# apachepinot/pinot

Hardware: AMD Instinct MI355X
Metric: rows scanned/sec, 1B-row segment filter+groupby (3 predicates, SUM/MAX GROUP BY g1) (higher is better)
Workload: dtype int64; 1 GPU; 1 segment(s) x 1000000000 rows, one per GPU; SELECT g1, SUM(m), MAX(m) FROM gpuBench WHERE c_inv1 IN (0,1,2,3) AND c_inv2 IN (0,1) AND r_int BETWEEN 250000 AND 749999 GROUP BY g1 ORDER BY g1 LIMIT 1000; query=cfg3, parallelism=segment-per-gpu x1, merge=none (1 segment), entries_scanned_in_filter=249990290

## Files before the change

pinot_amd/csrc/pg_kernels_spec.hip:

```cpp
#define PG_WAVES_PER_BLOCK 12
#define PG_KERNEL template <int PG_NOT_INSTANTIATED> static
#include "pg_kernels.hip"

#define SPEC_LOADERS 4
#ifndef SPEC_TILES
#define SPEC_TILES 2
#endif
#ifndef SPEC_SETS
#define SPEC_SETS 2
#endif
#define SPEC_CONSUMERS 8
#define SPEC_OFF_LIN 0u
#define SPEC_OFF_RNG 256u
#define SPEC_OFF_VAL (256u + 2048u)
#define SPEC_OFF_G0 (256u + 2048u + 8192u)
extern "C" const int pg_spec_waves_per_block = PG_WAVES_PER_BLOCK;
extern "C" int pg_spec_stage_bytes(int bits0, int bits1) { return SPEC_TILES * (((int)SPEC_OFF_G0 + bits0 * 256 + 16 + (bits1 > 0 ? bits1 * 256 + 16 : 0) + 15) & ~15); }

DEVFN void spec_barrier() {
  __builtin_amdgcn_fence(__ATOMIC_RELEASE, "workgroup", "local");
  __builtin_amdgcn_s_barrier();
  __builtin_amdgcn_fence(__ATOMIC_ACQUIRE, "workgroup", "local");
}

template <typename T> DEVFN const GAS T* spec_sgpr_ptr(const void* ptr) {
  const uint64_t v = (uint64_t)ptr;
  const uint32_t lo = (uint32_t)__builtin_amdgcn_readfirstlane((int)(uint32_t)v), hi = (uint32_t)__builtin_amdgcn_readfirstlane((int)(uint32_t)(v >> 32));
  return (const GAS T*)(((uint64_t)hi << 32) | (uint64_t)lo);
}

template <int W> struct SpecCol;
template <> struct SpecCol<0> {};
template <> struct SpecCol<32> { u32x4 r[2]; };
template <> struct SpecCol<24> { u32x4 lo; u32x2 hi; };
template <> struct SpecCol<16> { u32x4 lo; };
template <> struct SpecCol<8> { u32x2 hi; };
constexpr uint32_t spec_img_tile_bytes(int W) { return (uint32_t)(PG_WAVE_DOCS / 8) * (uint32_t)W; }
template <int W> DEVFN void spec_load(SpecCol<W>& c, const uint8_t* base, int wt, int w, int lane) {
  if constexpr (W == 32) {
#pragma unroll
    for (int s = 0; s < 2; s++) {
      const uint8_t* row = base + (size_t)wt * (PG_WAVE_DOCS * 4) + (size_t)(4 * s + w) * 1024u;
      c.r[s] = ldnt((const GAS u32x4*)(spec_sgpr_ptr<uint8_t>(row) + (uint32_t)lane * 16u));
    }
  } else if constexpr (W != 0) {
    const uint8_t* tile = base + (size_t)wt * spec_img_tile_bytes(W);
    if constexpr (W >= 16) c.lo = ldnt((const GAS u32x4*)(spec_sgpr_ptr<uint8_t>(tile + (size_t)w * 1024u) + (uint32_t)lane * 16u));
    if constexpr (W != 16) c.hi = ldnt((const GAS u32x2*)(spec_sgpr_ptr<uint8_t>(tile + (W == 24 ? 4096u : 0u) + (size_t)w * 512u) + (uint32_t)lane * 8u));
  }
}
template <int W> DEVFN void spec_unpack(const SpecCol<W>& c, uint32_t (&a)[4], uint32_t (&b)[4]) {
  if constexpr (W == 32) {
    a[0] = bswap32(c.r[0].x); a[1] = bswap32(c.r[0].y); a[2] = bswap32(c.r[0].z); a[3] = bswap32(c.r[0].w);
    b[0] = bswap32(c.r[1].x); b[1] = bswap32(c.r[1].y); b[2] = bswap32(c.r[1].z); b[3] = bswap32(c.r[1].w);
  } else if constexpr (W == 24) {
    a[0] = __builtin_amdgcn_perm(c.hi.x, c.lo.x, 0x0c040100u); a[1] = __builtin_amdgcn_perm(c.hi.x, c.lo.x, 0x0c050302u);
    a[2] = __builtin_amdgcn_perm(c.hi.x, c.lo.y, 0x0c060100u); a[3] = __builtin_amdgcn_perm(c.hi.x, c.lo.y, 0x0c070302u);
    b[0] = __builtin_amdgcn_perm(c.hi.y, c.lo.z, 0x0c040100u); b[1] = __builtin_amdgcn_perm(c.hi.y, c.lo.z, 0x0c050302u);
    b[2] = __builtin_amdgcn_perm(c.hi.y, c.lo.w, 0x0c060100u); b[3] = __builtin_amdgcn_perm(c.hi.y, c.lo.w, 0x0c070302u);
  } else if constexpr (W == 16) {
    a[0] = c.lo.x & 0xFFFFu; a[1] = c.lo.x >> 16; a[2] = c.lo.y & 0xFFFFu; a[3] = c.lo.y >> 16;
    b[0] = c.lo.z & 0xFFFFu; b[1] = c.lo.z >> 16; b[2] = c.lo.w & 0xFFFFu; b[3] = c.lo.w >> 16;
  } else if constexpr (W == 8) {
#pragma unroll
    for (int e = 0; e < 4; e++) { a[e] = (c.hi.x >> (8 * e)) & 0xFFu; b[e] = (c.hi.y >> (8 * e)) & 0xFFu; }
  }
}
template <int SW, int VW> struct SpecTile {
  SpecCol<SW> scan;
  SpecCol<VW> val;
  u32x4 grp;
};
template <int SW, int VW> struct SpecStage { SpecTile<SW, VW> tile[SPEC_TILES]; uint32_t post[8]; uint32_t tail; };
template <int NG> struct SpecQuad {
  uint32_t lin, rng;
  u32x4 val;
  uint32_t win[NG][2];
};

template <int W> struct SpecWidth { static constexpr int value = W; };
template <int NG, bool HAS_INDEX, bool HAS_SCAN, bool HAS_TAIL = false, bool NARROW = false>
__device__ __forceinline__ void spec_body(const PgQueryPlan& p) {
  extern __shared__ __attribute__((aligned(16))) uint64_t smem[];
  __shared__ uint32_t s_stat[PG_MAX_STATS];
  const int t = threadIdx.x;
  const int lane = t & 63;
  const int wave = uniform(t >> 6);
  int64_t* lds_table = reinterpret_cast<int64_t*>(smem);
  if (t < PG_MAX_STATS) s_stat[t] = 0;
  const uint32_t real_slots = (uint32_t)p.n_groups * (uint32_t)p.replicas;
  const uint32_t table_slots = real_slots + 64u;
  for (int o = 0; o < p.n_ops; o++) {
    const int64_t ident = pg_acc_identity(p.ops[o].fn, p.ops[o].is_float);
    for (uint32_t i = t; i < table_slots; i += PG_BLOCK) lds_table[(size_t)o * table_slots + i] = ident;
  }
  const uint32_t bits0 = (uint32_t)p.gcols[0].bits, bits1 = NG > 1 ? (uint32_t)p.gcols[NG - 1].bits : 0u;
  const uint32_t off_g1 = SPEC_OFF_G0 + bits0 * 256u + 16u;
  const uint32_t tile_bytes = (off_g1 + (NG > 1 ? bits1 * 256u + 16u : 0u) + 15u) & ~15u;
  const uint32_t stage_bytes = tile_bytes * SPEC_TILES;
  uint8_t* stage0 = reinterpret_cast<uint8_t*>(smem) + (((size_t)p.n_ops * table_slots * 8u + 15u) & ~(size_t)15u);
  const CAS PgScanLeaf& L = cptr(p.scans)[HAS_SCAN ? p.fast_scan : 0];
  const int grid = (int)gridDim.x;
  const int n_mine = (int)blockIdx.x < p.n_wtiles ? (p.n_wtiles - (int)blockIdx.x + grid - 1) / grid : 0;
  const int n_stages = (n_mine + SPEC_TILES - 1) / SPEC_TILES;
  __syncthreads();

  if (wave < SPEC_LOADERS) {
    const int w = wave;
    const uint8_t* const xdata = p.srcs[p.pipe_src].data;
    const uint8_t* const simg = NARROW ? p.spec_simg : nullptr;
    const uint8_t* const vimg = NARROW ? p.spec_vimg : nullptr;
    const uint32_t img_slo = NARROW ? p.spec_slo : 0u, img_sspan = NARROW ? p.spec_sspan : 0u, img_vmin = NARROW ? (uint32_t)p.spec_vmin : 0u;
    const bool img_sempty = NARROW && p.spec_sempty != 0;
    const int ggi = (w >> 1) < NG ? (w >> 1) : 0;
    const uint8_t* const gdata = p.gcols[ggi].data;
    const uint32_t gbits = (uint32_t)p.gcols[ggi].bits;
    const uint32_t goff = (uint32_t)(w & 1) * 1024u + (uint32_t)lane * 16u;
    const uint32_t geff = (w >> 1) < NG && goff < gbits * 256u ? goff : 0u;
    const uint8_t* dense_ptr[8];
    int dense_group[8];
#pragma unroll
    for (int j = 0; j < 8; j++) { dense_ptr[j] = HAS_INDEX ? p.dense_ptr[j] : nullptr; dense_group[j] = HAS_INDEX ? p.dense_group[j] : 0; }
    const int dense_groups = p.dense_groups, dense_excl = p.dense_excl;
    const uint8_t* const pipe_tail = HAS_TAIL ? p.pipe_tail : nullptr;
    const int num_docs = p.num_docs;
    const bool scan_pushed = p.fast_scan_pushed != 0;
   auto loaders = [&](auto scan_w, auto val_w) __attribute__((always_inline)) {
    constexpr int SW = HAS_SCAN ? decltype(scan_w)::value : 0, VW = decltype(val_w)::value;
    const RangeI32 r32 = !HAS_SCAN ? RangeI32{0, 0u, false} : (SW == 32 ? make_range_i32(L.lo, L.hi) : RangeI32{(int32_t)img_slo, img_sspan, img_sempty});
    const uint8_t* sdata = !HAS_SCAN ? nullptr : (SW == 32 ? L.data : simg);
    const uint8_t* vdata = VW == 32 ? xdata : vimg;
    const uint32_t vmin = VW == 32 ? 0u : img_vmin;
    uint32_t ld_cand = 0;
    auto issue = [&](int sidx, SpecStage<SW, VW>& st) __attribute__((always_inline)) {
#pragma unroll
      for (int tt = 0; tt < SPEC_TILES; tt++) {
        const int i = sidx * SPEC_TILES + tt;
        const int wt = (int)blockIdx.x + (i < n_mine ? i : n_mine - 1) * grid;
        SpecTile<SW, VW>& tl = st.tile[tt];
        __builtin_amdgcn_sched_barrier(0);
        spec_load<SW>(tl.scan, sdata, wt, w, lane);
        spec_load<VW>(tl.val, vdata, wt, w, lane);
        __builtin_amdgcn_sched_barrier(0);
        {
          const uint8_t* base = gdata + (size_t)wt * (size_t)(PG_WAVE_DOCS / 8) * (size_t)gbits;
          tl.grp = ldnt((const GAS u32x4*)(spec_sgpr_ptr<uint8_t>(base) + geff));
        }
        __builtin_amdgcn_sched_barrier(0);
      }
      if (HAS_INDEX) {
        const int i = sidx * SPEC_TILES + (w % SPEC_TILES);
        const int wt = (int)blockIdx.x + (i < n_mine ? i : n_mine - 1) * grid;
#pragma unroll
        for (int j = 0; j < 8; j++) st.post[j] = *(const GAS uint32_t*)(spec_sgpr_ptr<uint8_t>(dense_ptr[j] + (size_t)wt * 256u) + (uint32_t)lane * 4u);
        __builtin_amdgcn_sched_barrier(0);
      }
      if (HAS_TAIL) {
        const int i = sidx * SPEC_TILES + (w % SPEC_TILES);
        const int wt = (int)blockIdx.x + (i < n_mine ? i : n_mine - 1) * grid;
        st.tail = *(const GAS uint32_t*)(spec_sgpr_ptr<uint8_t>(pipe_tail + (size_t)wt * 256u) + (uint32_t)lane * 4u);
        __builtin_amdgcn_sched_barrier(0);
      }
    };
    auto publish = [&](uint8_t* stage, const SpecStage<SW, VW>& st) __attribute__((always_inline)) {
#ifdef PG_SPEC_NO_PUBLISH
      {
        uint32_t acc = 0;
#pragma unroll
        for (int tt = 0; tt < SPEC_TILES; tt++) {
          uint32_t a[4] = {0u, 0u, 0u, 0u}, b[4] = {0u, 0u, 0u, 0u};
          spec_unpack<SW>(st.tile[tt].scan, a, b); acc += a[0] ^ b[3];
          spec_unpack<VW>(st.tile[tt].val, a, b); acc += a[0] ^ b[3];
          acc += st.tile[tt].grp.x;
        }
        if (acc == 0x12345678u) *reinterpret_cast<uint32_t*>(stage) = acc;
        return;
      }
#endif
#pragma unroll
      for (int tt = 0; tt < SPEC_TILES; tt++) {
        uint8_t* buf = stage + (uint32_t)tt * tile_bytes;
        const SpecTile<SW, VW>& tl = st.tile[tt];
        if (HAS_SCAN) {
          uint32_t q[2][4];
          spec_unpack<SW>(tl.scan, q[0], q[1]);
#pragma unroll
          for (int s = 0; s < 2; s++) {
            uint32_t m = (uint32_t)in_range_i32(r32, (int32_t)q[s][0]) | ((uint32_t)in_range_i32(r32, (int32_t)q[s][1]) << 1) |
                         ((uint32_t)in_range_i32(r32, (int32_t)q[s][2]) << 2) | ((uint32_t)in_range_i32(r32, (int32_t)q[s][3]) << 3);
            m = r32.empty ? 0u : m;
            *reinterpret_cast<uint32_t*>(buf + SPEC_OFF_RNG + (uint32_t)(4 * s + w) * 256u + (uint32_t)lane * 4u) = m;
          }
        }
        {
          uint32_t q[2][4];
          spec_unpack<VW>(tl.val, q[0], q[1]);
#pragma unroll
          for (int s = 0; s < 2; s++) {
            u32x4 v;
            v.x = q[s][0] + vmin; v.y = q[s][1] + vmin; v.z = q[s][2] + vmin; v.w = q[s][3] + vmin;
            *reinterpret_cast<u32x4*>(buf + SPEC_OFF_VAL + (uint32_t)(4 * s + w) * 1024u + (uint32_t)lane * 16u) = v;
          }
        }
        *reinterpret_cast<u32x4*>(buf + (ggi == 0 ? SPEC_OFF_G0 : off_g1) + geff) = tl.grp;
      }
    };
    auto publish_lin = [&](uint8_t* stage, const SpecStage<SW, VW>& st, int sidx) __attribute__((always_inline)) {
      if (w >= SPEC_TILES) return;
      const int i = sidx * SPEC_TILES + w;
      const int wt = (int)blockIdx.x + i * grid;
      const int64_t rem = i < n_mine ? (int64_t)num_docs - (int64_t)wt * PG_WAVE_DOCS : 0;
      const int32_t n_valid = rem >= PG_WAVE_DOCS ? PG_WAVE_DOCS : (rem > 0 ? (int32_t)rem : 0);
      uint32_t lin = valid_lin_mask(n_valid, lane);
      if (HAS_INDEX) {
        uint32_t grp[4] = {0u, 0u, 0u, 0u};
#pragma unroll
        for (int j = 0; j < 8; j++) {
          const int gj = dense_group[j];
#pragma unroll
          for (int k = 0; k < 4; k++) grp[k] |= gj == k ? st.post[j] : 0u;
        }
#pragma unroll
        for (int k = 0; k < 4; k++)
          if (k < dense_groups) lin &= ((dense_excl >> k) & 1) ? ~grp[k] : grp[k];
      }
      *reinterpret_cast<uint32_t*>(stage + (uint32_t)w * tile_bytes + SPEC_OFF_LIN + (uint32_t)lane * 4u) = HAS_TAIL ? lin & st.tail : lin;
      ld_cand += (uint32_t)__popc(lin);
    };
    constexpr int SETS = HAS_SCAN ? SPEC_SETS : 2 * SPEC_SETS;
    SpecStage<SW, VW> st[SETS];
    auto buf_of = [&](int sg) __attribute__((always_inline)) { return stage0 + (uint32_t)(sg & 1) * stage_bytes; };
    if (n_stages > 0) {
#pragma unroll
      for (int k = 0; k < SETS; k++) issue(k, st[k]);
    }
    int s = 0;
    for (; s + SETS - 1 < n_stages; s += SETS) {
#pragma unroll
      for (int k = 0; k < SETS; k++) {
        publish(buf_of(s + k), st[k]);
        publish_lin(buf_of(s + k), st[k], s + k);
        issue(s + k + SETS, st[k]);
        spec_barrier();
      }
    }
#pragma unroll
    for (int k = 0; k < SETS - 1; k++)
      if (s + k < n_stages) {
        publish(buf_of(s + k), st[k]);
        publish_lin(buf_of(s + k), st[k], s + k);
        spec_barrier();
      }
    const uint32_t csum = wave_sum_u32(ld_cand);
    if (HAS_SCAN && !scan_pushed && lane == 0 && csum) atomicAdd(&s_stat[L.stat_slot], csum);
   };
    if constexpr (!NARROW) {
      loaders(SpecWidth<32>{}, SpecWidth<32>{});
    } else {
      const int sb = uniform(p.spec_sbits), vb = uniform(p.spec_vbits);
      auto with_scan = [&](auto scan_w) __attribute__((always_inline)) {
        switch (vb) {
          case 8: loaders(scan_w, SpecWidth<8>{}); break;
          case 16: loaders(scan_w, SpecWidth<16>{}); break;
          case 24: loaders(scan_w, SpecWidth<24>{}); break;
          default: loaders(scan_w, SpecWidth<32>{}); break;
        }
      };
      switch (sb) {
        case 8: with_scan(SpecWidth<8>{}); break;
        case 16: with_scan(SpecWidth<16>{}); break;
        case 24: with_scan(SpecWidth<24>{}); break;
        default: with_scan(SpecWidth<32>{}); break;
      }
    }
  } else {
    const int c = wave - SPEC_LOADERS;
    const uint32_t R = (uint32_t)p.replicas;
    const uint32_t rep = (uint32_t)t & (R - 1u);
    const uint32_t stride = table_slots;
    const uint32_t trash_slot = real_slots + (uint32_t)lane;
    const uint32_t q = (uint32_t)c * 64u + (uint32_t)lane;
    const uint32_t nib = ((uint32_t)lane & 7u) * 4u;
    uint32_t my_matched = 0;
    const int n_ops = uniform(p.n_ops);
    uint64_t ops_code = 0;
    for (int o = 0; o < n_ops; o++) {
      const PgAccOp op = p.ops[uniform(o)];
      ops_code |= (uint64_t)(op.src < 0 ? 0u : (op.fn == PG_ACC_SUM ? 1u : (op.fn == PG_ACC_MIN ? 2u : 3u))) << (2 * o);
    }
    ops_code = ((uint64_t)(uint32_t)uniform((int)(uint32_t)(ops_code >> 32)) << 32) | (uint64_t)(uint32_t)uniform((int)(uint32_t)ops_code);
    const int has_out_words = uniform(p.out_words != nullptr ? 1 : 0);
    auto fetch = [&](const uint8_t* buf, SpecQuad<NG>& d) __attribute__((always_inline)) {
      d.lin = *reinterpret_cast<const uint32_t*>(buf + SPEC_OFF_LIN + (q >> 3) * 4u);
      d.rng = HAS_SCAN ? *reinterpret_cast<const uint32_t*>(buf + SPEC_OFF_RNG + q * 4u) : 0xFu;
      d.val = *reinterpret_cast<const u32x4*>(buf + SPEC_OFF_VAL + q * 16u);
#pragma unroll
      for (int gi = 0; gi < NG; gi++) {
        const uint32_t di = __umul24(4u * q, (uint32_t)p.gcols[gi].bits) >> 5;
        const uint32_t* win = reinterpret_cast<const uint32_t*>(buf + (gi == 0 ? SPEC_OFF_G0 : off_g1)) + di;
        d.win[gi][0] = win[0]; d.win[gi][1] = win[1];
      }
    };
    auto aggregate = [&](const SpecQuad<NG> (&d)[SPEC_TILES], int sidx) __attribute__((always_inline)) {
      constexpr int ND = 4 * SPEC_TILES;
      uint32_t slot[ND];
      int32_t v[ND];
#pragma unroll
      for (int tt = 0; tt < SPEC_TILES; tt++) {
        const int i = sidx * SPEC_TILES + tt;
        const uint32_t cand = (d[tt].lin >> nib) & 0xFu;
        const uint32_t m = d[tt].rng & cand;
        my_matched += (uint32_t)__popc(m);
        if (has_out_words && i < n_mine) {
          const int wt = (int)blockIdx.x + i * grid;
          const uint32_t word = or_reduce8(m << nib);
          if ((lane & 7) == 0) reinterpret_cast<uint32_t*>(p.out_words)[(int64_t)wt * 64 + (int64_t)(q >> 3)] = word;
        }
#ifndef PG_SPEC_NO_TABLE
#pragma unroll
        for (int e = 0; e < 4; e++) slot[4 * tt + e] = rep;
#pragma unroll
        for (int gi = 0; gi < NG; gi++) {
          const PgGroupCol& gc = p.gcols[gi];
          const uint32_t bits = (uint32_t)gc.bits, mask = (1u << gc.bits) - 1u;
          const uint32_t mult = (uint32_t)gc.mult * R;
          uint32_t dv[4];
          decode_packed_quad<true>(d[tt].win[gi], q, bits, mask, dv);
#pragma unroll
          for (int e = 0; e < 4; e++) slot[4 * tt + e] += __umul24(dv[e], mult);
        }
#pragma unroll
        for (int e = 0; e < 4; e++) slot[4 * tt + e] = ((m >> e) & 1u) ? slot[4 * tt + e] : trash_slot;
        v[4 * tt + 0] = (int32_t)d[tt].val.x; v[4 * tt + 1] = (int32_t)d[tt].val.y; v[4 * tt + 2] = (int32_t)d[tt].val.z; v[4 * tt + 3] = (int32_t)d[tt].val.w;
#endif
      }
#ifdef PG_SPEC_NO_TABLE
      return;
#endif
      for (int o = 0; o < n_ops; o++) {
        const uint32_t code = (uint32_t)(ops_code >> (2 * o)) & 3u;
        int64_t* base = lds_table + (size_t)o * stride;
        if (code == 0u) {
#pragma unroll
          for (int e = 0; e < ND; e++) atomicAdd(reinterpret_cast<unsigned long long*>(base + slot[e]), 1ULL);
        } else if (code == 1u) {
#pragma unroll
          for (int e = 0; e < ND; e++) atomicAdd(reinterpret_cast<unsigned long long*>(base + slot[e]), (unsigned long long)(int64_t)v[e]);
        } else if (code == 2u) {
#pragma unroll
          for (int e = 0; e < ND; e++) atomicMin(reinterpret_cast<long long*>(base + slot[e]), (long long)v[e]);
        } else {
#pragma unroll
          for (int e = 0; e < ND; e++) atomicMax(reinterpret_cast<long long*>(base + slot[e]), (long long)v[e]);
        }
      }
    };
    auto fetch_stage = [&](int sidx, SpecQuad<NG> (&d)[SPEC_TILES]) __attribute__((always_inline)) {
      const uint8_t* stage = stage0 + (uint32_t)(sidx & 1) * stage_bytes;
#pragma unroll
      for (int tt = 0; tt < SPEC_TILES; tt++) fetch(stage + (uint32_t)tt * tile_bytes, d[tt]);
    };
    auto aggregate_stage = [&](int sidx, const SpecQuad<NG> (&d)[SPEC_TILES]) __attribute__((always_inline)) {
#ifdef PG_SPEC_NO_CONSUME
      return;
#endif
#ifdef PG_SPEC_FETCH_ONLY
      {
        uint32_t acc = 0;
#pragma unroll
        for (int tt = 0; tt < SPEC_TILES; tt++) { acc += d[tt].lin ^ d[tt].rng ^ d[tt].val.x ^ d[tt].val.w; for (int gi = 0; gi < NG; gi++) acc += d[tt].win[gi][0] ^ d[tt].win[gi][1]; }
        if (acc == 0x12345678u) my_matched++;
        return;
      }
#endif
      aggregate(d, sidx);
    };
    SpecQuad<NG> da[SPEC_TILES], db[SPEC_TILES];
    if (n_stages > 0) {
      spec_barrier();
#ifndef PG_SPEC_NO_CONSUME
      fetch_stage(0, da);
#endif
    }
    for (int s = 0; s < n_stages; s += 2) {
      if (s + 1 < n_stages) {
        spec_barrier();
#ifndef PG_SPEC_NO_CONSUME
        fetch_stage(s + 1, db);
#endif
      }
      aggregate_stage(s, da);
      if (s + 1 < n_stages) {
        if (s + 2 < n_stages) {
          spec_barrier();
#ifndef PG_SPEC_NO_CONSUME
          fetch_stage(s + 2, da);
#endif
        }
        aggregate_stage(s + 1, db);
      }
    }
    const uint32_t wsum = wave_sum_u32(my_matched);
    if (lane == 0 && wsum) atomicAdd(&s_stat[0], wsum);
  }
  __syncthreads();
  if (t < PG_MAX_STATS && s_stat[t]) atomicAdd(&p.stats[t], (unsigned long long)s_stat[t]);
  {
    const int R = p.replicas, groups = p.n_groups;
    int64_t* out = p.partials + (int64_t)blockIdx.x * ((int64_t)p.n_ops * groups);
    for (int o = 0; o < p.n_ops; o++) {
      const int fn = p.ops[uniform(o)].fn;
      for (int gq = t; gq < groups; gq += PG_BLOCK) {
        const int64_t* src = lds_table + (size_t)o * table_slots + (size_t)gq * R;
        int64_t acc = src[0];
        if (fn == PG_ACC_COUNT || fn == PG_ACC_SUM) { for (int r = 1; r < R; r++) acc += src[r]; }
        else if (fn == PG_ACC_MIN) { for (int r = 1; r < R; r++) acc = src[r] < acc ? src[r] : acc; }
        else { for (int r = 1; r < R; r++) acc = src[r] > acc ? src[r] : acc; }
        out[(size_t)o * groups + gq] = acc;
      }
    }
  }
}
#define PG_SPEC_KERNEL(NAME, IDX, SCAN) \
  extern "C" __global__ void __launch_bounds__(PG_BLOCK) NAME(const PgQueryPlan p) { \
    if (p.n_group_cols == 1) spec_body<1, IDX, SCAN>(p); \
    else spec_body<2, IDX, SCAN>(p); \
  }
PG_SPEC_KERNEL(pg_spec_none, false, false)
PG_SPEC_KERNEL(pg_spec_scan, false, true)
PG_SPEC_KERNEL(pg_spec_index, true, false)
#undef PG_SPEC_KERNEL
extern "C" __global__ void __launch_bounds__(PG_BLOCK) pg_fast_i32range_s(const PgQueryPlan p) {
  if (p.n_group_cols == 1) spec_body<1, true, true, false, true>(p);
  else spec_body<2, true, true, false, true>(p);
}
extern "C" __global__ void __launch_bounds__(PG_BLOCK) pg_fast_i32range_st(const PgQueryPlan p) {
  if (p.n_group_cols == 1) spec_body<1, true, true, true, true>(p);
  else spec_body<2, true, true, true, true>(p);
}
```

Measured before the change: 841.7 billion rows/s.

## Double loader waves and split tiles across loaders with specialized role variants

Raises the loader wave count from 4 to 8, giving 16 waves per block. Each loader now handles a subset of tiles (SPEC_LT), so more wavefronts keep global loads in flight. Loader roles are specialized at compile time: only the waves that need them load posting lists, tail masks and group columns. The number of dense posting slots loaded is trimmed to the ones actually used, and those loads become non-temporal. Larger blocks and more role variants may lower occupancy and increase code size.

```diff
diff --git a/pinot_amd/csrc/pg_kernels_spec.hip b/pinot_amd/csrc/pg_kernels_spec.hip
--- a/pinot_amd/csrc/pg_kernels_spec.hip
+++ b/pinot_amd/csrc/pg_kernels_spec.hip
@@ -1,15 +1,22 @@
-#define PG_WAVES_PER_BLOCK 12
+#ifndef SPEC_LOADERS
+#define SPEC_LOADERS 8
+#endif
+#define SPEC_CONSUMERS 8
+#define PG_WAVES_PER_BLOCK (SPEC_LOADERS + SPEC_CONSUMERS)
 #define PG_KERNEL template <int PG_NOT_INSTANTIATED> static
 #include "pg_kernels.hip"
 
-#define SPEC_LOADERS 4
+#ifdef PG_SPEC_LOADS_ONLY
+#define PG_SPEC_NO_CONSUME
+#endif
 #ifndef SPEC_TILES
 #define SPEC_TILES 2
 #endif
 #ifndef SPEC_SETS
 #define SPEC_SETS 2
 #endif
-#define SPEC_CONSUMERS 8
+#define SPEC_LT (SPEC_TILES * 4 / SPEC_LOADERS)
+static_assert((SPEC_LOADERS == 4 || SPEC_LOADERS == 8) && SPEC_TILES <= 4 && SPEC_LT >= 1 && SPEC_LT * SPEC_LOADERS == SPEC_TILES * 4, "loaders per tile");
 #define SPEC_OFF_LIN 0u
 #define SPEC_OFF_RNG 256u
 #define SPEC_OFF_VAL (256u + 2048u)
@@ -71,7 +78,7 @@
   SpecCol<VW> val;
   u32x4 grp;
 };
-template <int SW, int VW> struct SpecStage { SpecTile<SW, VW> tile[SPEC_TILES]; uint32_t post[8]; uint32_t tail; };
+template <int SW, int VW> struct SpecStage { SpecTile<SW, VW> tile[SPEC_LT]; uint32_t post[8]; uint32_t tail; };
 template <int NG> struct SpecQuad {
   uint32_t lin, rng;
   u32x4 val;
@@ -106,27 +113,48 @@
   __syncthreads();
 
   if (wave < SPEC_LOADERS) {
+#ifdef PG_SPEC_LOADER_PRIO
+    __builtin_amdgcn_s_setprio(1);
+#endif
     const int w = wave;
+    const int wr = w & 3;
+    const int t0 = (w >> 2) * SPEC_LT;
+    const int lin_t = 3 - wr;
+    const bool is_lin = lin_t >= t0 && lin_t < t0 + SPEC_LT;
     const uint8_t* const xdata = p.srcs[p.pipe_src].data;
     const uint8_t* const simg = NARROW ? p.spec_simg : nullptr;
     const uint8_t* const vimg = NARROW ? p.spec_vimg : nullptr;
     const uint32_t img_slo = NARROW ? p.spec_slo : 0u, img_sspan = NARROW ? p.spec_sspan : 0u, img_vmin = NARROW ? (uint32_t)p.spec_vmin : 0u;
     const bool img_sempty = NARROW && p.spec_sempty != 0;
-    const int ggi = (w >> 1) < NG ? (w >> 1) : 0;
+    const int ggi = (wr >> 1) < NG ? (wr >> 1) : 0;
     const uint8_t* const gdata = p.gcols[ggi].data;
     const uint32_t gbits = (uint32_t)p.gcols[ggi].bits;
-    const uint32_t goff = (uint32_t)(w & 1) * 1024u + (uint32_t)lane * 16u;
-    const uint32_t geff = (w >> 1) < NG && goff < gbits * 256u ? goff : 0u;
+    const uint32_t goff = (uint32_t)(wr & 1) * 1024u + (uint32_t)lane * 16u;
+    const uint32_t geff = goff < gbits * 256u ? goff : 0u;
+    const bool has_grp = (wr >> 1) < NG && (uint32_t)(wr & 1) * 1024u < gbits * 256u;
     const uint8_t* dense_ptr[8];
     int dense_group[8];
 #pragma unroll
     for (int j = 0; j < 8; j++) { dense_ptr[j] = HAS_INDEX ? p.dense_ptr[j] : nullptr; dense_group[j] = HAS_INDEX ? p.dense_group[j] : 0; }
     const int dense_groups = p.dense_groups, dense_excl = p.dense_excl;
+    int n_slots = 1;
+#pragma unroll
+    for (int j = 1; j < 8; j++)
+      if (HAS_INDEX && (dense_ptr[j] != dense_ptr[0] || dense_group[j] != dense_group[0])) n_slots = j + 1;
+    n_slots = uniform(n_slots);
+    uint32_t dense_in[8][4];
+#pragma unroll
+    for (int j = 0; j < 8; j++) {
+#pragma unroll
+      for (int k = 0; k < 4; k++) dense_in[j][k] = HAS_INDEX && dense_group[j] == k ? ~0u : 0u;
+    }
     const uint8_t* const pipe_tail = HAS_TAIL ? p.pipe_tail : nullptr;
     const int num_docs = p.num_docs;
     const bool scan_pushed = p.fast_scan_pushed != 0;
-   auto loaders = [&](auto scan_w, auto val_w) __attribute__((always_inline)) {
+   auto loaders = [&](auto scan_w, auto val_w, auto lin_role, auto grp_role) __attribute__((always_inline)) {
     constexpr int SW = HAS_SCAN ? decltype(scan_w)::value : 0, VW = decltype(val_w)::value;
+    constexpr int NP = decltype(lin_role)::value;
+    constexpr bool LIN = NP != 0, GRP = decltype(grp_role)::value != 0;
     const RangeI32 r32 = !HAS_SCAN ? RangeI32{0, 0u, false} : (SW == 32 ? make_range_i32(L.lo, L.hi) : RangeI32{(int32_t)img_slo, img_sspan, img_sempty});
     const uint8_t* sdata = !HAS_SCAN ? nullptr : (SW == 32 ? L.data : simg);
     const uint8_t* vdata = VW == 32 ? xdata : vimg;
@@ -134,52 +162,75 @@
     uint32_t ld_cand = 0;
     auto issue = [&](int sidx, SpecStage<SW, VW>& st) __attribute__((always_inline)) {
 #pragma unroll
-      for (int tt = 0; tt < SPEC_TILES; tt++) {
-        const int i = sidx * SPEC_TILES + tt;
+      for (int tt = 0; tt < SPEC_LT; tt++) {
+        const int i = sidx * SPEC_TILES + t0 + tt;
         const int wt = (int)blockIdx.x + (i < n_mine ? i : n_mine - 1) * grid;
         SpecTile<SW, VW>& tl = st.tile[tt];
         __builtin_amdgcn_sched_barrier(0);
-        spec_load<SW>(tl.scan, sdata, wt, w, lane);
-        spec_load<VW>(tl.val, vdata, wt, w, lane);
+        spec_load<SW>(tl.scan, sdata, wt, wr, lane);
+        spec_load<VW>(tl.val, vdata, wt, wr, lane);
         __builtin_amdgcn_sched_barrier(0);
-        {
+        if constexpr (GRP) {
           const uint8_t* base = gdata + (size_t)wt * (size_t)(PG_WAVE_DOCS / 8) * (size_t)gbits;
           tl.grp = ldnt((const GAS u32x4*)(spec_sgpr_ptr<uint8_t>(base) + geff));
         }
         __builtin_amdgcn_sched_barrier(0);
       }
-      if (HAS_INDEX) {
-        const int i = sidx * SPEC_TILES + (w % SPEC_TILES);
+      if constexpr (LIN && HAS_INDEX) {
+        const int i = sidx * SPEC_TILES + lin_t;
         const int wt = (int)blockIdx.x + (i < n_mine ? i : n_mine - 1) * grid;
 #pragma unroll
-        for (int j = 0; j < 8; j++) st.post[j] = *(const GAS uint32_t*)(spec_sgpr_ptr<uint8_t>(dense_ptr[j] + (size_t)wt * 256u) + (uint32_t)lane * 4u);
+        for (int j = 0; j < NP; j++) st.post[j] = ldnt((const GAS uint32_t*)(spec_sgpr_ptr<uint8_t>(dense_ptr[j] + (size_t)wt * 256u) + (uint32_t)lane * 4u));
         __builtin_amdgcn_sched_barrier(0);
       }
-      if (HAS_TAIL) {
-        const int i = sidx * SPEC_TILES + (w % SPEC_TILES);
+      if constexpr (LIN && HAS_TAIL) {
+        const int i = sidx * SPEC_TILES + lin_t;
         const int wt = (int)blockIdx.x + (i < n_mine ? i : n_mine - 1) * grid;
         st.tail = *(const GAS uint32_t*)(spec_sgpr_ptr<uint8_t>(pipe_tail + (size_t)wt * 256u) + (uint32_t)lane * 4u);
         __builtin_amdgcn_sched_barrier(0);
       }
     };
     auto publish = [&](uint8_t* stage, const SpecStage<SW, VW>& st) __attribute__((always_inline)) {
+#ifdef PG_SPEC_LOADS_ONLY
+      {
+        uint32_t acc = 0;
+#pragma unroll
+        for (int tt = 0; tt < SPEC_LT; tt++) {
+          const SpecTile<SW, VW>& tl = st.tile[tt];
+          if constexpr (SW == 32) acc ^= tl.scan.r[0].x ^ tl.scan.r[1].x;
+          if constexpr (SW == 24 || SW == 16) acc ^= tl.scan.lo.x;
+          if constexpr (SW == 24 || SW == 8) acc ^= tl.scan.hi.x;
+          if constexpr (VW == 32) acc ^= tl.val.r[0].x ^ tl.val.r[1].x;
+          if constexpr (VW == 24 || VW == 16) acc ^= tl.val.lo.x;
+          if constexpr (VW == 24 || VW == 8) acc ^= tl.val.hi.x;
+          if constexpr (GRP) acc ^= tl.grp.x;
+        }
+        if constexpr (LIN && HAS_INDEX) {
+#pragma unroll
+          for (int j = 0; j < NP; j++) acc ^= st.post[j];
+        }
+        if constexpr (LIN && HAS_TAIL) acc ^= st.tail;
+        if (acc == 0x12345678u) *reinterpret_cast<uint32_t*>(stage) = acc;
+        return;
+      }
+#endif
 #ifdef PG_SPEC_NO_PUBLISH
       {
         uint32_t acc = 0;
 #pragma unroll
-        for (int tt = 0; tt < SPEC_TILES; tt++) {
+        for (int tt = 0; tt < SPEC_LT; tt++) {
           uint32_t a[4] = {0u, 0u, 0u, 0u}, b[4] = {0u, 0u, 0u, 0u};
           spec_unpack<SW>(st.tile[tt].scan, a, b); acc += a[0] ^ b[3];
           spec_unpack<VW>(st.tile[tt].val, a, b); acc += a[0] ^ b[3];
-          acc += st.tile[tt].grp.x;
+          if constexpr (GRP) acc += st.tile[tt].grp.x;
         }
         if (acc == 0x12345678u) *reinterpret_cast<uint32_t*>(stage) = acc;
         return;
       }
 #endif
 #pragma unroll
-      for (int tt = 0; tt < SPEC_TILES; tt++) {
-        uint8_t* buf = stage + (uint32_t)tt * tile_bytes;
+      for (int tt = 0; tt < SPEC_LT; tt++) {
+        uint8_t* buf = stage + (uint32_t)(t0 + tt) * tile_bytes;
         const SpecTile<SW, VW>& tl = st.tile[tt];
         if (HAS_SCAN) {
           uint32_t q[2][4];
@@ -189,25 +240,32 @@
             uint32_t m = (uint32_t)in_range_i32(r32, (int32_t)q[s][0]) | ((uint32_t)in_range_i32(r32, (int32_t)q[s][1]) << 1) |
                          ((uint32_t)in_range_i32(r32, (int32_t)q[s][2]) << 2) | ((uint32_t)in_range_i32(r32, (int32_t)q[s][3]) << 3);
             m = r32.empty ? 0u : m;
-            *reinterpret_cast<uint32_t*>(buf + SPEC_OFF_RNG + (uint32_t)(4 * s + w) * 256u + (uint32_t)lane * 4u) = m;
+            *reinterpret_cast<uint32_t*>(buf + SPEC_OFF_RNG + (uint32_t)(4 * s + wr) * 256u + (uint32_t)lane * 4u) = m;
           }
         }
         {
           uint32_t q[2][4];
           spec_unpack<VW>(tl.val, q[0], q[1]);
+          if (VW != 32 && vmin != 0u) {
+#pragma unroll
+            for (int e = 0; e < 4; e++) { q[0][e] += vmin; q[1][e] += vmin; }
+          }
 #pragma unroll
           for (int s = 0; s < 2; s++) {
             u32x4 v;
-            v.x = q[s][0] + vmin; v.y = q[s][1] + vmin; v.z = q[s][2] + vmin; v.w = q[s][3] + vmin;
-            *reinterpret_cast<u32x4*>(buf + SPEC_OFF_VAL + (uint32_t)(4 * s + w) * 1024u + (uint32_t)lane * 16u) = v;
+            v.x = q[s][0]; v.y = q[s][1]; v.z = q[s][2]; v.w = q[s][3];
+            *reinterpret_cast<u32x4*>(buf + SPEC_OFF_VAL + (uint32_t)(4 * s + wr) * 1024u + (uint32_t)lane * 16u) = v;
           }
         }
-        *reinterpret_cast<u32x4*>(buf + (ggi == 0 ? SPEC_OFF_G0 : off_g1) + geff) = tl.grp;
+        if constexpr (GRP) *reinterpret_cast<u32x4*>(buf + (ggi == 0 ? SPEC_OFF_G0 : off_g1) + geff) = tl.grp;
       }
     };
     auto publish_lin = [&](uint8_t* stage, const SpecStage<SW, VW>& st, int sidx) __attribute__((always_inline)) {
-      if (w >= SPEC_TILES) return;
-      const int i = sidx * SPEC_TILES + w;
+#ifdef PG_SPEC_LOADS_ONLY
+      return;
+#endif
+      if constexpr (!LIN) return;
+      const int i = sidx * SPEC_TILES + lin_t;
       const int wt = (int)blockIdx.x + i * grid;
       const int64_t rem = i < n_mine ? (int64_t)num_docs - (int64_t)wt * PG_WAVE_DOCS : 0;
       const int32_t n_valid = rem >= PG_WAVE_DOCS ? PG_WAVE_DOCS : (rem > 0 ? (int32_t)rem : 0);
@@ -215,16 +273,15 @@
       if (HAS_INDEX) {
         uint32_t grp[4] = {0u, 0u, 0u, 0u};
 #pragma unroll
-        for (int j = 0; j < 8; j++) {
-          const int gj = dense_group[j];
-#pragma unroll
-          for (int k = 0; k < 4; k++) grp[k] |= gj == k ? st.post[j] : 0u;
+        for (int j = 0; j < NP; j++) {
+#pragma unroll
+          for (int k = 0; k < 4; k++) grp[k] |= st.post[j] & dense_in[j][k];
         }
 #pragma unroll
         for (int k = 0; k < 4; k++)
           if (k < dense_groups) lin &= ((dense_excl >> k) & 1) ? ~grp[k] : grp[k];
       }
-      *reinterpret_cast<uint32_t*>(stage + (uint32_t)w * tile_bytes + SPEC_OFF_LIN + (uint32_t)lane * 4u) = HAS_TAIL ? lin & st.tail : lin;
+      *reinterpret_cast<uint32_t*>(stage + (uint32_t)lin_t * tile_bytes + SPEC_OFF_LIN + (uint32_t)lane * 4u) = HAS_TAIL ? lin & st.tail : lin;
       ld_cand += (uint32_t)__popc(lin);
     };
     constexpr int SETS = HAS_SCAN ? SPEC_SETS : 2 * SPEC_SETS;
@@ -254,16 +311,27 @@
     const uint32_t csum = wave_sum_u32(ld_cand);
     if (HAS_SCAN && !scan_pushed && lane == 0 && csum) atomicAdd(&s_stat[L.stat_slot], csum);
    };
+    auto with_roles = [&](auto scan_w, auto val_w) __attribute__((always_inline)) {
+      auto with_grp = [&](auto lin_role) __attribute__((always_inline)) {
+        constexpr bool lin = decltype(lin_role)::value != 0;
+        if (lin ? NG > 1 : uniform(has_grp ? 1 : 0) != 0) loaders(scan_w, val_w, lin_role, SpecWidth<1>{});
+        else loaders(scan_w, val_w, lin_role, SpecWidth<0>{});
+      };
+      if (!uniform(is_lin ? 1 : 0)) with_grp(SpecWidth<0>{});
+      else if (!HAS_INDEX || n_slots <= 4) with_grp(SpecWidth<4>{});
+      else if (n_slots <= 6) with_grp(SpecWidth<6>{});
+      else with_grp(SpecWidth<8>{});
+    };
     if constexpr (!NARROW) {
-      loaders(SpecWidth<32>{}, SpecWidth<32>{});
+      with_roles(SpecWidth<32>{}, SpecWidth<32>{});
     } else {
       const int sb = uniform(p.spec_sbits), vb = uniform(p.spec_vbits);
       auto with_scan = [&](auto scan_w) __attribute__((always_inline)) {
         switch (vb) {
-          case 8: loaders(scan_w, SpecWidth<8>{}); break;
-          case 16: loaders(scan_w, SpecWidth<16>{}); break;
-          case 24: loaders(scan_w, SpecWidth<24>{}); break;
-          default: loaders(scan_w, SpecWidth<32>{}); break;
+          case 8: with_roles(scan_w, SpecWidth<8>{}); break;
+          case 16: with_roles(scan_w, SpecWidth<16>{}); break;
+          case 24: with_roles(scan_w, SpecWidth<24>{}); break;
+          default: with_roles(scan_w, SpecWidth<32>{}); break;
         }
       };
       switch (sb) {
```

Measured after the change: 876.2 billion rows/s, median of 6. 1.04x the previous value.
